# leonsick/s2d

Measured on AMD Instinct MI355X. Metric: clip-frames/sec fwd+loss, R50 M2F-Video T=8 720p Q=100, higher is better.
Workload: dtype f32 (f16x3 MFMA for dense contractions); 1 GPU; KDVideoMaskFormer fwd+loss (student+teacher fwd, GT+KD VideoSetCriterion), c4: 2 clips/GPU x T=8 x 720x1280, Q=100, P=160000, N=10 sparse GT instances/clip, encoder dropout 0.3; clips_per_gpu=2, frames_per_clip=8, parallelism=dp1 (clips sharded, no collective), streams=2

## Files before the change

s2d_amd/csrc/loss.hip:

```cpp
#include "common.h"
#include "class_select.h"

namespace {

__device__ __forceinline__ uint64_t mix64(uint64_t z)
{
    z += 0x9E3779B97F4A7C15ull;
    z = (z ^ (z >> 30)) * 0xBF58476D1CE4E5B9ull;
    z = (z ^ (z >> 27)) * 0x94D049BB133111EBull;
    return z ^ (z >> 31);
}
__device__ __forceinline__ uint32_t hash32(uint32_t x)
{
    x ^= x >> 16; x *= 0x7feb352du; x ^= x >> 15; x *= 0x846ca68bu; x ^= x >> 16;
    return x;
}
__device__ __forceinline__ uint32_t rand_key(uint64_t seed, uint64_t stream)
{
    return (uint32_t)mix64(seed ^ mix64(stream * 0xD1342543DE82EF95ull));
}
__device__ __forceinline__ uint32_t rand_u_bits(uint32_t key, uint32_t i) { return hash32(key + i); }
__device__ __forceinline__ uint32_t rand_v_bits(uint32_t a)
{
    uint32_t b = a * 0x9E3779B1u;
// ... 48 lines not shown
        int c = 0;
        for (int j = 0; j < Q; ++j)
            if (keep[j] && c < Nmax) kept[b * Nmax + c++] = j;
        count[b] = c;
    }
}

__global__ __launch_bounds__(256) void kd_upsample_kernel(const float *__restrict__ ml, int ldq, int T, int hm, int wm, int H,
                                                          int W, int Nmax, const int *__restrict__ count,
                                                          const int *__restrict__ kept, uint8_t *__restrict__ tgt,
                                                          int *__restrict__ nonempty)
{
    __shared__ int kq[128];
    __shared__ unsigned int anyset[128];
    const int bt = blockIdx.z, b = bt / T, t = bt % T;
    const int Y = blockIdx.y, X = blockIdx.x * 256 + threadIdx.x;
    const int cnt = count[b];
    if (threadIdx.x < 128) {
        kq[threadIdx.x] = threadIdx.x < cnt ? kept[b * Nmax + threadIdx.x] : 0;
        anyset[threadIdx.x] = 0u;
    }
    __syncthreads();
    if (X < W) {
        float sy = ((float)hm / H) * (Y + 0.5f) - 0.5f; if (sy < 0.f) sy = 0.f;
        float sx = ((float)wm / W) * (X + 0.5f) - 0.5f; if (sx < 0.f) sx = 0.f;
        const int y0 = (int)sy, x0 = (int)sx, y1 = y0 + (y0 < hm - 1 ? 1 : 0), x1 = x0 + (x0 < wm - 1 ? 1 : 0);
        const float ly = sy - y0, lx = sx - x0, hy = 1.f - ly, hx = 1.f - lx;
        const float *fr = ml + ((long)b * T + t) * hm * wm * ldq;
        const float *r00 = fr + ((long)y0 * wm + x0) * ldq, *r01 = fr + ((long)y0 * wm + x1) * ldq;
        const float *r10 = fr + ((long)y1 * wm + x0) * ldq, *r11 = fr + ((long)y1 * wm + x1) * ldq;
        for (int k = 0; k < cnt; ++k) {
            const int q = kq[k];
            const float val = hy * (hx * r00[q] + lx * r01[q]) + ly * (hx * r10[q] + lx * r11[q]);
            const uint8_t m = val > 0.f ? 1 : 0;
            tgt[((((long)b * Nmax + k) * T + t) * H + Y) * W + X] = m;
            if (m) anyset[k] = 1u;
        }
    }
    __syncthreads();
    if (threadIdx.x < cnt && anyset[threadIdx.x]) nonempty[((long)b * Nmax + threadIdx.x) * T + t] = 1;
}

constexpr int KDT_H = 16, KDT_W = 256, KDT_SH = 8, KDT_SW = 72, KDT_KC = 8;
__global__ __launch_bounds__(256) void kd_upsample_tile_kernel(const float *__restrict__ ml, int ldq, int T, int hm, int wm, int H,
                                                               int W, int Nmax, const int *__restrict__ count,
                                                               const int *__restrict__ kept, uint8_t *__restrict__ tgt,
                                                               int *__restrict__ nonempty)
{
    __shared__ int kq[128];
    __shared__ unsigned int anyset[128];
    __shared__ float src[KDT_KC][KDT_SH][KDT_SW];
    const int bt = blockIdx.z, b = bt / T, t = bt % T;
    const int Y0 = blockIdx.y * KDT_H, X0 = blockIdx.x * KDT_W;
    const int cnt = count[b];
    if (threadIdx.x < 128) {
        kq[threadIdx.x] = threadIdx.x < cnt ? kept[b * Nmax + threadIdx.x] : 0;
        anyset[threadIdx.x] = 0u;
    }
    auto srcpos = [](int o, int n_out, int n_in, int &i0, int &i1, float &l) {
        float s = ((float)n_in / n_out) * (o + 0.5f) - 0.5f; if (s < 0.f) s = 0.f;
        i0 = (int)s; i1 = i0 + (i0 < n_in - 1 ? 1 : 0); l = s - i0;
    };
    int ya, yb_, xa, xb_; float dummy;
    srcpos(Y0, H, hm, ya, yb_, dummy);
    srcpos(X0, W, wm, xa, xb_, dummy);
    const float *fr = ml + ((long)b * T + t) * hm * wm * ldq;
    const int xg = X0 + 4 * (threadIdx.x & 63);
    int x0[4], x1[4]; float lx[4];
#pragma unroll
    for (int e = 0; e < 4; ++e) srcpos(min(xg + e, W - 1), W, wm, x0[e], x1[e], lx[e]);
    __syncthreads();
    for (int k0 = 0; k0 < cnt; k0 += KDT_KC) {
        const int kc = min(KDT_KC, cnt - k0);
        for (int i = threadIdx.x; i < KDT_SH * KDT_SW * KDT_KC; i += 256) {
            const int kk = i % KDT_KC, pix = i / KDT_KC, sx = pix % KDT_SW, sy = pix / KDT_SW;
            const int gy = min(ya + sy, hm - 1), gx = min(xa + sx, wm - 1);
            if (kk < kc) src[kk][sy][sx] = fr[((long)gy * wm + gx) * ldq + kq[k0 + kk]];
        }
        __syncthreads();
#pragma unroll
        for (int pss = 0; pss < 4; ++pss) {
            const int Y = Y0 + (threadIdx.x >> 6) + 4 * pss;
            if (Y >= H || xg >= W) continue;
            int y0, y1; float ly;
            srcpos(Y, H, hm, y0, y1, ly);
            const float hy = 1.f - ly;
            for (int kk = 0; kk < kc; ++kk) {
                unsigned int word = 0u;
#pragma unroll
                for (int e = 0; e < 4; ++e) {
                    const float hx = 1.f - lx[e];
                    const float val = hy * (hx * src[kk][y0 - ya][x0[e] - xa] + lx[e] * src[kk][y0 - ya][x1[e] - xa]) +
                                      ly * (hx * src[kk][y1 - ya][x0[e] - xa] + lx[e] * src[kk][y1 - ya][x1[e] - xa]);
                    word |= (val > 0.f ? 1u : 0u) << (8 * e);
                }
                *reinterpret_cast<unsigned int *>(tgt + ((((long)b * Nmax + k0 + kk) * T + t) * H + Y) * W + xg) = word;
                if (word) anyset[k0 + kk] = 1u;
            }
        }
        __syncthreads();
    }
    if (threadIdx.x < cnt && anyset[threadIdx.x]) atomicOr(&nonempty[((long)b * Nmax + threadIdx.x) * T + t], 1);
}

constexpr int NE_CHUNKS = 8;
__global__ __launch_bounds__(256) void nonempty_kernel(const uint8_t *__restrict__ tgt, const int *__restrict__ count, int Nmax,
                                                       int T, long HW, int *__restrict__ nonempty)
{
    const int plane = blockIdx.x;
    const int n = (plane / T) % Nmax, b = plane / (T * Nmax);
    if (n >= count[b]) return;
    const uint8_t *p = tgt + (long)plane * HW;
    int any = 0;
    const long n16 = HW / 16, per = (n16 + NE_CHUNKS - 1) / NE_CHUNKS;
    const long lo = blockIdx.y * per, hi = min(lo + per, n16);
    const uint4 *p4 = reinterpret_cast<const uint4 *>(p);
    for (long i = lo + threadIdx.x; i < hi; i += 256) {
        const uint4 v = p4[i];
        any |= (v.x | v.y | v.z | v.w) != 0u;
    }
    if (blockIdx.y == 0)
        for (long i = n16 * 16 + threadIdx.x; i < HW; i += 256) any |= p[i] != 0;
    any = __syncthreads_or(any);
    if (threadIdx.x == 0 && any) atomicOr(&nonempty[plane], 1);
}

struct LossParams {
    const float *ml;
    const uint8_t *tgt;
    const int *tgt_count;
    const int *nonempty;
    const int *idx_q, *idx_t;
    const int *n_match;
    const float *coords_over;
    const float *coords_rand;
    uint64_t seed;
    int NL, B, Q, ldq, T, hm, wm, H, W, Nmax, maxm, n_over, n_unc, n_rand, drop;
    float world_size;
    int *active, *rank;
    int *list;
    int *lcount;
    float *mq;
    unsigned int *hist;
    unsigned int *prefix;
    int *krem;
    unsigned int *tie;
    float *part;
    int chunks;
    float *xbuf;
    unsigned int *tpack;
    int bits_global;
    int xcap;
    int *pbound;
};

__device__ __forceinline__ uint64_t key_row(const LossParams &p, long rowid)
{
    if (p.NL == 0) return (uint64_t)rowid;
    const long per = (long)p.maxm * p.T;
    const long lb = rowid / per;
    return (uint64_t)(lb * ((long)p.Q * p.T) + (rowid - lb * per));
}

constexpr int PB_STRIDE = 9;
struct VRange {
    float v0, dv;
};

__global__ void row_prep_kernel(LossParams p)
{
    const int layer = blockIdx.x;
    const int rows_l = p.B * p.maxm * p.T;
    __shared__ int base;
    if (threadIdx.x == 0) base = 0;
    __syncthreads();
    for (int r0 = 0; r0 < rows_l; r0 += blockDim.x) {
        const int r = r0 + threadIdx.x;
        int act = 0;
        if (r < rows_l) {
            const int t = r % p.T, s = (r / p.T) % p.maxm, b = r / (p.T * p.maxm);
            const int prob = layer * p.B + b;
            if (s < p.n_match[prob]) {
                const int n = p.idx_t[(long)prob * p.maxm + s];
                act = p.drop ? p.nonempty[((long)b * p.Nmax + n) * p.T + t] : 1;
            }
        }
        __shared__ int wsum[4];
        const unsigned long long m = __ballot(act);
        const int lane = threadIdx.x & 63, wv = threadIdx.x >> 6;
        const int inw = __popcll(m & ((1ull << lane) - 1ull));
        if (lane == 0) wsum[wv] = __popcll(m);
        __syncthreads();
        int off = base;
        for (int w = 0; w < wv; ++w) off += wsum[w];
        if (r < rows_l) {
            const long rowid = (long)layer * rows_l + r;
            p.active[rowid] = act;
            p.rank[rowid] = off + inw;
        }
        __syncthreads();
        if (threadIdx.x == 0) base += wsum[0] + wsum[1] + wsum[2] + wsum[3];
        __syncthreads();
    }
    if (threadIdx.x == 0) p.lcount[layer] = base;
}

__global__ void row_list_kernel(LossParams p)
{
    const int layer = blockIdx.x;
    const int rows_l = p.B * p.maxm * p.T;
    int base = 0;
    for (int l = 0; l < layer; ++l) base += p.lcount[l];
    for (int r = threadIdx.x; r < rows_l; r += blockDim.x) {
        const long rowid = (long)layer * rows_l + r;
        if (p.active[rowid]) p.list[base + p.rank[rowid]] = (int)rowid;
    }
    if (layer == p.NL - 1 && threadIdx.x == 0) p.lcount[p.NL] = base + p.lcount[layer];
}

__device__ int binomial_inv(int N, double p, double U);
__global__ __launch_bounds__(256) void row_strata_kernel(LossParams p, int nparts, int rpp)
{
    const int n = p.lcount[p.NL];
    const int wave = (blockIdx.x * 256 + threadIdx.x) >> 6, nwaves = gridDim.x * 4;
    for (int li = wave; li < n; li += nwaves) {
        const long rowid = p.list[li];
        int *pb = p.pbound + rowid * PB_STRIDE;
        int rem = p.n_over, at = 0;
        double mass = 1.0;
        for (int j = 0; j < nparts; ++j) {
            if ((threadIdx.x & 63) == 0) pb[j] = at;
            const double ya = j == 0 ? -0.5 : (double)(j * rpp), yb = j == nparts - 1 ? (double)p.hm - 0.5 : (double)((j + 1) * rpp);
            const double pj = (yb - ya) / (double)p.hm;
            int nj = rem;
            if (j < nparts - 1) {
                const uint64_t h = mix64(p.seed ^ mix64((key_row(p, rowid) * 16u + (uint64_t)j) * 0xD1342543DE82EF95ull + 0x5851F42D4C957F2Dull));
                const double U = (double)(h >> 11) * (1.0 / 9007199254740992.0);
                const double pc = pj / mass;
                nj = binomial_inv(rem, pc < 1.0 ? pc : 1.0, U);
            }
            at += nj; rem -= nj; mass -= pj;
        }
        if ((threadIdx.x & 63) == 0) pb[nparts] = at;
    }
}

__global__ void rng_points_prep_kernel(int *list, int nrows)
{
    const int i = blockIdx.x * 256 + threadIdx.x;
    if (i < nrows) list[i] = i;
    else if (i == nrows) list[i] = nrows;
}
__device__ __forceinline__ void over_point_rng(uint32_t key0, int i, const int *pb, const float *v0, const float *dv, int nparts, float &u, float &v);
__device__ __forceinline__ VRange part_vrange(int j, int nparts, int rpp, int hm);
__global__ void rng_points_kernel(LossParams p, int nparts, int rpp, float *__restrict__ uv)
{
    const int row = blockIdx.y, i = blockIdx.x * 256 + threadIdx.x;
    __shared__ float s_v0[PB_STRIDE], s_dv[PB_STRIDE];
    if ((int)threadIdx.x < nparts) { const VRange vr = part_vrange(threadIdx.x, nparts, rpp, p.hm); s_v0[threadIdx.x] = vr.v0; s_dv[threadIdx.x] = vr.dv; }
    __syncthreads();
    if (i >= p.n_over) return;
    float u, v;
    over_point_rng(rand_key(p.seed, (uint64_t)row * 2), i, p.pbound + (long)row * PB_STRIDE, s_v0, s_dv, nparts, u, v);
    uv[((long)row * p.n_over + i) * 2] = u;
    uv[((long)row * p.n_over + i) * 2 + 1] = v;
}

__global__ __launch_bounds__(256) void gather_rows_kernel(LossParams p)
{
    __shared__ float tile[64][129];
    const int prob = blockIdx.z, t = blockIdx.y, pix0 = blockIdx.x * 64;
    const int layer = prob / p.B, b = prob % p.B;
    const int hw = p.hm * p.wm;
    const int nm = p.n_match[prob];
    const long row_base = (((long)layer * p.B + b) * p.maxm) * p.T;
    bool any = false;
    for (int s = 0; s < nm; ++s) any = any || p.active[row_base + (long)s * p.T + t];
    if (!any) return;
    const float *src = p.ml + (((long)prob * p.T + t) * hw + pix0) * p.ldq;
    const int npix = min(64, hw - pix0);
    const int l4 = p.ldq >> 2;
    f32x4 v[8];
    const int tot = npix * l4;
#pragma unroll
    for (int k = 0; k < 8; ++k) {
        const int e = threadIdx.x + 256 * k;
        if (e < tot) v[k] = *reinterpret_cast<const f32x4 *>(src + (long)e * 4);
    }
#pragma unroll
    for (int k = 0; k < 8; ++k) {
        const int e = threadIdx.x + 256 * k;
        if (e < tot) {
            const int px = e / l4, q = (e - px * l4) * 4;
            if (q < 128) { tile[px][q] = v[k][0]; tile[px][q + 1] = v[k][1]; tile[px][q + 2] = v[k][2]; tile[px][q + 3] = v[k][3]; }
        }
    }
    __syncthreads();
    const int lane = threadIdx.x & 63, wv = threadIdx.x >> 6;
    for (int s = wv; s < nm; s += 4) {
        const long rowid = row_base + (long)s * p.T + t;
        if (!p.active[rowid]) continue;
        const int q = p.idx_q[(long)prob * p.maxm + s];
        if (lane < npix) p.mq[rowid * hw + pix0 + lane] = tile[lane][q];
    }
}

// ... 118 lines not shown
        reinterpret_cast<f32x4 *>(sm + (long)(nr + 1) * wp)[i] = z;
    }
    for (int i = threadIdx.x; i < nr; i += LTHREADS) {
        *reinterpret_cast<f32x4 *>(sm + (long)(i + 1) * wp) = z;
        *reinterpret_cast<f32x4 *>(sm + (long)(i + 1) * wp + PADC + wm) = z;
    }
    const f32x4 *src = reinterpret_cast<const f32x4 *>(map + (long)r0 * wm);
    for (int e = threadIdx.x; e < nr * w4; e += LTHREADS) {
        const int row = e / w4, c4 = e - row * w4;
        *reinterpret_cast<f32x4 *>(sm + (long)(row + 1) * wp + PADC + 4 * c4) = src[e];
    }
}

__device__ __forceinline__ float sample_part_padded(const float *__restrict__ sm, int wp, int r0, float x, float y, int x0, int y0)
{
    const float fx = x - x0, fy = y - y0;
    const float *b = sm + (y0 - r0 + 1) * wp + x0 + PADC;
    float acc = b[0] * ((1.f - fx) * (1.f - fy));
    acc += b[1] * (fx * (1.f - fy));
    acc += b[wp] * ((1.f - fx) * fy);
    acc += b[wp + 1] * (fx * fy);
    return acc;
}

__device__ __forceinline__ float sample_part(const float *__restrict__ sm, int hm, int wm, int r0, int nr, float x, float y, int x0, int y0)
{
    const int x1 = x0 + 1, y1 = y0 + 1;
    const float fx = x - x0, fy = y - y0;
    const float wxa = (x0 >= 0) ? 1.f - fx : 0.f, wxb = (x1 < wm) ? fx : 0.f;
    const float wya = (y0 >= 0) ? 1.f - fy : 0.f, wyb = (y1 < hm) ? fy : 0.f;
    const int xa = max(x0, 0), xb = min(x1, wm - 1);
    const int ya = min(max(y0 - r0, 0), nr - 1) * wm, yb = min(max(min(y1, hm - 1) - r0, 0), nr - 1) * wm;
    float acc = sm[ya + xa] * (wxa * wya);
    acc += sm[ya + xb] * (wxb * wya);
    acc += sm[yb + xa] * (wxa * wyb);
    acc += sm[yb + xb] * (wxb * wyb);
    return acc;
}

#ifndef S2D_LOSS_DBG
#define S2D_LOSS_DBG 0
#endif
template <int LEVEL>
__global__ __launch_bounds__(LTHREADS) void hist_kernel(LossParams p)
{
    extern __shared__ __attribute__((aligned(16))) float smem[];
    __shared__ int hq_idx[LTHREADS / 64][128];
    __shared__ float hq_y[LTHREADS / 64][128];
    constexpr int nb = LEVEL == 0 ? 2048 : 1024;
    const PartGeom g = part_geom(p.hm, p.wm);
    unsigned int *h = reinterpret_cast<unsigned int *>(smem);
    float *sm = smem + 2048;
    PartIter it(p, g.nparts, LEVEL == 0 ? 0 : p.xcap);
    long rowid; int part, li;
    while (it.next(p, rowid, part, li)) {
        __syncthreads();
        for (int i = threadIdx.x; i < nb; i += LTHREADS) h[i] = 0u;
        const int r0 = part * g.rows_per_part;
        const int nr = min(g.rows_per_part + 1, p.hm - r0);
        const float *cr = coord_rows(p, rowid, true);
        const bool padded = cr == nullptr;
        const int wp = p.wm + 2 * PADC;
        if (padded) stage_part_padded(p.mq + rowid * p.hm * p.wm, p.wm, r0, nr, sm);
        else stage_part(p.mq + rowid * p.hm * p.wm, p.wm, r0, nr, sm);
        __syncthreads();
        const unsigned int pre = LEVEL > 0 ? p.prefix[rowid] : 0u;
        const uint32_t key0 = rand_key(p.seed, key_row(p, rowid) * 2);
        const int ylo = part == 0 ? -1 : r0, yhi = r0 + g.rows_per_part;
        auto tally = [&](int i, float xv) {
            const unsigned int key = __float_as_uint(fabsf(xv));
            if (LEVEL == 0 && li < p.xcap && !(S2D_LOSS_DBG & 4)) p.xbuf[(long)li * (p.n_over + p.n_rand) + i] = xv;
            if ((S2D_LOSS_DBG & 1) && LEVEL == 0) { if (key == 0x12345u) h[0] = 1u; return; }
            if (LEVEL == 0) atomicAdd(&h[key >> 20], 1u);
            else if (LEVEL == 1) { if ((key >> 20) == (pre >> 20)) atomicAdd(&h[(key >> 10) & 1023u], 1u); }
            else { if ((key >> 10) == (pre >> 10)) atomicAdd(&h[key & 1023u], 1u); }
        };
        if (!cr) {
            const int *pb = p.pbound + rowid * PB_STRIDE;
            const int lo = pb[part], hi = pb[part + 1];
            const VRange vr = part_vrange(part, g.nparts, g.rows_per_part, p.hm);
            const int y0max = min(yhi, p.hm) - 1;
#pragma unroll 2
            for (int i = lo + (int)threadIdx.x; i < hi; i += LTHREADS) {
                const uint32_t ra_ = rand_u_bits(key0, (uint32_t)i);
                const float u = (float)(ra_ >> 8) * (1.0f / 16777216.0f);
                const float v = fmaf((float)(rand_v_bits(ra_) >> 8) * (1.0f / 16777216.0f), vr.dv, vr.v0);
                const float y = ((2.f * v - 1.f + 1.f) * p.hm - 1.f) * 0.5f;
                const float x = ((2.f * u - 1.f + 1.f) * p.wm - 1.f) * 0.5f;
                const int y0 = min(max((int)floorf(y), ylo), y0max);
                if (S2D_LOSS_DBG & 2) tally(i, x * y + (float)y0); else
                tally(i, sample_part_padded(sm, wp, r0, x, y, (int)floorf(x), y0));
            }
        } else {
            const int lane = threadIdx.x & 63, wv = threadIdx.x >> 6;
            int *qi = hq_idx[wv];
            float *qy = hq_y[wv];
            int qn = 0;
            auto heavy = [&](int i, float y) {
                const float u = cr[2 * i];
                const float x = ((2.f * u - 1.f + 1.f) * p.wm - 1.f) * 0.5f;
                tally(i, sample_part(sm, p.hm, p.wm, r0, nr, x, y, (int)floorf(x), (int)floorf(y)));
            };
            const int iters = (p.n_over + LTHREADS - 1) / LTHREADS;
            for (int k = 0; k < iters; ++k) {
                const int i = k * LTHREADS + threadIdx.x;
                const bool live = i < p.n_over;
                const int ic = live ? i : p.n_over - 1;
                const float v = cr[2 * ic + 1];
                const float y = ((2.f * v - 1.f + 1.f) * p.hm - 1.f) * 0.5f;
                const int y0 = (int)floorf(y);
                const bool own = live && y0 >= ylo && y0 < yhi;
                const unsigned long long m = __ballot(own);
                if (own) {
                    const int pos = qn + (int)__popcll(m & ((1ull << lane) - 1ull));
                    qi[pos] = i; qy[pos] = y;
                }
                qn += (int)__popcll(m);
                if (qn >= 64) {
                    heavy(qi[lane], qy[lane]);
                    const int rest = qn - 64;
                    int ti = 0; float ty = 0.f;
                    if (lane < rest) { ti = qi[64 + lane]; ty = qy[64 + lane]; }
                    if (lane < rest) { qi[lane] = ti; qy[lane] = ty; }
                    qn = rest;
                }
            }
            if (lane < qn) heavy(qi[lane], qy[lane]);
        }
        if (LEVEL == 0 && li < p.xcap) {
            const float *cr2 = coord_rows(p, rowid, false);
            const uint32_t key1 = rand_key(p.seed, key_row(p, rowid) * 2 + 1);
            for (int i = threadIdx.x; i < p.n_rand; i += LTHREADS) {
                float u, v;
                if (cr2) { u = cr2[2 * i]; v = cr2[2 * i + 1]; }
                else {
                    const uint32_t ra_ = rand_u_bits(key1, (uint32_t)i);
                    u = (float)(ra_ >> 8) * (1.0f / 16777216.0f);
                    v = (float)(rand_v_bits(ra_) >> 8) * (1.0f / 16777216.0f);
                }
                const float y = ((2.f * v - 1.f + 1.f) * p.hm - 1.f) * 0.5f;
                const float x = ((2.f * u - 1.f + 1.f) * p.wm - 1.f) * 0.5f;
                const int y0 = (int)floorf(y);
                if (y0 >= ylo && y0 < yhi)
                    p.xbuf[(long)li * (p.n_over + p.n_rand) + p.n_over + i] =
                        padded ? sample_part_padded(sm, wp, r0, x, y, (int)floorf(x), y0) : sample_part(sm, p.hm, p.wm, r0, nr, x, y, (int)floorf(x), y0);
            }
        }
        __syncthreads();
        for (int i = threadIdx.x; i < nb; i += LTHREADS)
            if (h[i]) atomicAdd(&p.hist[rowid * 2048 + i], h[i]);
    }
}

template <int LEVEL>
__global__ __launch_bounds__(256) void hist_stream_kernel(LossParams p)
{
    __shared__ unsigned int h[1024];
    constexpr int SCH = 8;
    const int nrows = min(p.lcount[p.NL], p.xcap);
    for (int w = blockIdx.x; w < nrows * SCH; w += gridDim.x) {
        const int li = w / SCH, chunk = w % SCH;
        const long rowid = p.list[li];
        __syncthreads();
        for (int i = threadIdx.x; i < 1024; i += 256) h[i] = 0u;
        __syncthreads();
        const unsigned int pre = p.prefix[rowid];
        const float *xb = p.xbuf + (long)li * (p.n_over + p.n_rand);
        const int per = ((p.n_over + SCH - 1) / SCH + 3) & ~3;
        const int i0 = chunk * per, i1 = min(p.n_over, i0 + per);
        for (int i = i0 + threadIdx.x * 4; i < i1; i += 256 * 4) {
            const f32x4 v = *reinterpret_cast<const f32x4 *>(xb + i);
#pragma unroll
            for (int j = 0; j < 4; ++j) {
                if (i + j >= i1) break;
                const unsigned int key = __float_as_uint(fabsf(v[j]));
                if (LEVEL == 1) { if ((key >> 20) == (pre >> 20)) atomicAdd(&h[(key >> 10) & 1023u], 1u); }
                else { if ((key >> 10) == (pre >> 10)) atomicAdd(&h[key & 1023u], 1u); }
            }
        }
        __syncthreads();
        for (int i = threadIdx.x; i < 1024; i += 256)
            if (h[i]) atomicAdd(&p.hist[rowid * 2048 + i], h[i]);
    }
}

template <bool COH = false>
__device__ __forceinline__ float sample_bits(const unsigned int *bits, int H, int W, float u, float v)
{
    const float gx = 2.f * u - 1.f, gy = 2.f * v - 1.f;
    const float x = ((gx + 1.f) * W - 1.f) * 0.5f, y = ((gy + 1.f) * H - 1.f) * 0.5f;
    const int x0 = (int)floorf(x), y0 = (int)floorf(y), x1 = x0 + 1, y1 = y0 + 1;
    const float fx = x - x0, fy = y - y0;
    const float wxa = (x0 >= 0 && x0 < W) ? 1.f - fx : 0.f, wxb = (x1 >= 0 && x1 < W) ? fx : 0.f;
    const float wya = (y0 >= 0 && y0 < H) ? 1.f - fy : 0.f, wyb = (y1 >= 0 && y1 < H) ? fy : 0.f;
    const int xa = min(max(x0, 0), W - 1), xb = min(max(x1, 0), W - 1);
    const int ya = min(max(y0, 0), H - 1) * W, yb = min(max(y1, 0), H - 1) * W;
    auto bit = [&](int idx) {
        const unsigned int w = COH ? __hip_atomic_load(bits + (idx >> 5), __ATOMIC_RELAXED, __HIP_MEMORY_SCOPE_AGENT) : bits[idx >> 5];
        return (float)((w >> (idx & 31)) & 1u);
    };
    float acc = bit(ya + xa) * (wxa * wya);
    acc += bit(ya + xb) * (wxb * wya);
    acc += bit(yb + xa) * (wxa * wyb);
    acc += bit(yb + xb) * (wxb * wyb);
    return acc;
}

template <int LEVEL>
__global__ __launch_bounds__(256) void select_kernel(LossParams p)
{
    __shared__ unsigned int csum[256];
    if ((int)blockIdx.x >= p.lcount[p.NL]) return;
    const long rowid = p.list[blockIdx.x];
    const int nb = LEVEL == 0 ? 2048 : 1024, per = nb / 256;
    const int k = LEVEL == 0 ? p.n_unc : p.krem[rowid];
    unsigned int *h = p.hist + rowid * 2048;
    unsigned int loc[8], s = 0;
    for (int j = 0; j < per; ++j) { loc[j] = h[threadIdx.x * per + j]; s += loc[j]; }
    csum[threadIdx.x] = s;
    __syncthreads();
    if (threadIdx.x == 0) {
        unsigned int run = 0;
        for (int i = 0; i < 256; ++i) { const unsigned int c = csum[i]; csum[i] = run; run += c; }
    }
    __syncthreads();
    unsigned int before = csum[threadIdx.x];
    if (k == 0 && LEVEL == 0 && threadIdx.x == 0) { p.prefix[rowid] = 0u; p.krem[rowid] = 0; }
    for (int j = 0; j < per; ++j) {
        if (before < (unsigned)k && before + loc[j] >= (unsigned)k) {
            const unsigned int bin = threadIdx.x * per + j;
            const unsigned int pre = LEVEL == 0 ? 0u : p.prefix[rowid];
            p.prefix[rowid] = LEVEL == 0 ? (bin << 20) : LEVEL == 1 ? (pre | (bin << 10)) : (pre | bin);
            p.krem[rowid] = k - (int)before;
        }
        before += loc[j];
    }
    __syncthreads();
    for (int j = 0; j < per; ++j) h[threadIdx.x * per + j] = 0u;
}

__device__ __forceinline__ void acc_point(float x, float t, float &bce, float &sgt, float &sg, float &ts)
{
    const float e = __expf(-fabsf(x));
    const float inv = __builtin_amdgcn_rcpf(1.f + e);
    const float s = x >= 0.f ? inv : e * inv;
    bce += fmaxf(x, 0.f) - x * t + __logf(1.f + e);
    sgt += s * t; sg += s; ts += t;
}

__global__ __launch_bounds__(LTHREADS) void accumulate_kernel(LossParams p)
{
    extern __shared__ __attribute__((aligned(16))) float smem[];
    __shared__ float red[LTHREADS / 64][4];
    const PartGeom g = part_geom(p.hm, p.wm);
    float *sm = smem;
    const int rows_l = p.B * p.maxm * p.T;
    PartIter it(p, g.nparts, p.xcap);
    long rowid; int part, li;
    while (it.next(p, rowid, part, li)) {
        __syncthreads();
        const int r0 = part * g.rows_per_part;
        const int nr = min(g.rows_per_part + 1, p.hm - r0);
        stage_part(p.mq + rowid * p.hm * p.wm, p.wm, r0, nr, sm);
        __syncthreads();
        const int layer = (int)(rowid / rows_l);
        const int r = (int)(rowid % rows_l);
        const int t = r % p.T, s = (r / p.T) % p.maxm, b = r / (p.T * p.maxm);
        const int prob = layer * p.B + b;
        const int n = p.idx_t[(long)prob * p.maxm + s];
        const uint8_t *pl = p.tgt + (((long)b * p.Nmax + n) * p.T + t) * p.H * p.W;
        const unsigned int thr = p.prefix[rowid];
        const unsigned int take = (unsigned int)p.krem[rowid];
        const int ylo = part == 0 ? -1 : r0, yhi = r0 + g.rows_per_part;
        float bce = 0.f, sgt = 0.f, sg = 0.f, ts = 0.f;
#pragma unroll 1
        for (int pass = 0; pass < 2; ++pass) {
            const bool over = pass == 0;
            const float *cr = coord_rows(p, rowid, over);
            const uint32_t key0 = rand_key(p.seed, key_row(p, rowid) * 2 + (over ? 0 : 1));
            const bool strat = over && !cr;
            const int *pb = p.pbound + rowid * PB_STRIDE;
            const int ibeg = strat ? pb[part] : 0, cnt = strat ? pb[part + 1] : (over ? p.n_over : p.n_rand);
            const VRange vr = part_vrange(part, g.nparts, g.rows_per_part, p.hm);
            const int y0max = min(yhi, p.hm) - 1;
            for (int i0 = ibeg + (int)threadIdx.x; i0 < cnt; i0 += 4 * LTHREADS) {
                float xv[4], uu[4], vv[4];
                bool own[4];
#pragma unroll
                for (int j = 0; j < 4; ++j) {
                    const int i = i0 + j * LTHREADS;
                    const int ic = min(i, cnt - 1);
                    float u, v;
                    if (cr) { u = cr[2 * ic]; v = cr[2 * ic + 1]; }
                    else {
                        const uint32_t ra_ = rand_u_bits(key0, (uint32_t)ic);
                        u = (float)(ra_ >> 8) * (1.0f / 16777216.0f);
                        v = (float)(rand_v_bits(ra_) >> 8) * (1.0f / 16777216.0f);
                        if (strat) v = fmaf(v, vr.dv, vr.v0);
                    }
                    const float y = ((2.f * v - 1.f + 1.f) * p.hm - 1.f) * 0.5f;
                    const float x = ((2.f * u - 1.f + 1.f) * p.wm - 1.f) * 0.5f;
                    int y0 = (int)floorf(y);
                    if (strat) y0 = min(max(y0, ylo), y0max);
                    own[j] = i < cnt && y0 >= ylo && y0 < yhi;
                    xv[j] = sample_part(sm, p.hm, p.wm, r0, nr, x, y, (int)floorf(x), y0);
                    uu[j] = u; vv[j] = v;
                }
#pragma unroll
                for (int j = 0; j < 4; ++j) {
                    bool sel = own[j];
                    if (over && sel) {
                        const unsigned int key = __float_as_uint(fabsf(xv[j]));
                        sel = key < thr;
                        if (key == thr) sel = atomicAdd(&p.tie[rowid], 1u) < take;
                    }
                    if (sel) acc_point(xv[j], sample_plane(pl, p.H, p.W, uu[j], vv[j]), bce, sgt, sg, ts);
                }
            }
        }
        bce = wave_sum(bce); sgt = wave_sum(sgt); sg = wave_sum(sg); ts = wave_sum(ts);
        const int lane = threadIdx.x & 63, wv = threadIdx.x >> 6;
        if (lane == 0) { red[wv][0] = bce; red[wv][1] = sgt; red[wv][2] = sg; red[wv][3] = ts; }
        __syncthreads();
        if (threadIdx.x < 4) {
            const int j = threadIdx.x;
            float tot = 0.f;
#pragma unroll
            for (int w = 0; w < LTHREADS / 64; ++w) tot += red[w][j];
            p.part[(rowid * p.chunks + part) * 4 + j] = tot;
        }
    }
}

__global__ __launch_bounds__(256) void pack_planes_kernel(LossParams p)
{
    const long HW = (long)p.H * p.W, wpp = HW / 32;
    const int plane = blockIdx.y;
    const int n = (plane / p.T) % p.Nmax, b = plane / (p.T * p.Nmax);
    if (n >= min(p.tgt_count[b], p.Nmax)) return;
    const long wd = (long)blockIdx.x * 256 + threadIdx.x;
    if (wd >= wpp) return;
    const uint8_t *pl = p.tgt + (long)plane * HW;
    const uint4 a = reinterpret_cast<const uint4 *>(pl)[wd * 2], c = reinterpret_cast<const uint4 *>(pl)[wd * 2 + 1];
    const unsigned int ws[8] = {a.x, a.y, a.z, a.w, c.x, c.y, c.z, c.w};
    unsigned int out = 0u;
#pragma unroll
    for (int k = 0; k < 8; ++k) {
        const unsigned int w4 = ws[k];
        out |= ((w4 & 0xFFu) ? 1u : 0u) << (4 * k);
        out |= ((w4 & 0xFF00u) ? 1u : 0u) << (4 * k + 1);
        out |= ((w4 & 0xFF0000u) ? 1u : 0u) << (4 * k + 2);
        out |= ((w4 & 0xFF000000u) ? 1u : 0u) << (4 * k + 3);
    }
    p.tpack[(long)plane * wpp + wd] = out;
}

struct LossBwdArgs {
    float *gplane;
    float w_mask, w_dice;
    unsigned int *bit_scratch;
};
template <bool BWD, bool GBITS = BWD>
__global__ __launch_bounds__(LTHREADS) void accumulate_stream_kernel(LossParams p, LossBwdArgs ba)
{
    extern __shared__ __attribute__((aligned(16))) unsigned int tbits[];
    __shared__ float red[LTHREADS / 64][4];
    constexpr int TIECAP = 512;
    __shared__ unsigned int tie_n, tie_base, wtie[LTHREADS / 64];
    __shared__ int tie_idx[TIECAP], tie_sorted[TIECAP];
    __shared__ int cq_idx[LTHREADS / 64][128];
    __shared__ float cq_val[LTHREADS / 64][128];
    const int rows_l = p.B * p.maxm * p.T;
    const int nrows = min(p.lcount[p.NL], p.xcap);
    const long HW = (long)p.H * p.W;
    __shared__ float s_v0[PB_STRIDE], s_dv[PB_STRIDE];
    __shared__ int s_pb[PB_STRIDE];
    const PartGeom sg_ = part_geom(p.hm, p.wm);
    if ((int)threadIdx.x < sg_.nparts) { const VRange vr = part_vrange(threadIdx.x, sg_.nparts, sg_.rows_per_part, p.hm); s_v0[threadIdx.x] = vr.v0; s_dv[threadIdx.x] = vr.dv; }
    static_assert(GBITS || !BWD, "the backward keeps its gradient tile in the dynamic LDS");
    const unsigned int *tb = tbits;
    int *gh = reinterpret_cast<int *>(tbits);
    const float n_pts = (float)(p.n_unc + p.n_rand);
    const bool injected = p.coords_over != nullptr || p.coords_rand != nullptr;
    const float FX_CAP = injected ? fmaxf(n_pts, 1.f) : fminf(fmaxf(n_pts, 1.f), fmaxf(1024.f, 256.f * n_pts / (float)(p.hm * p.wm)));
    __shared__ unsigned int tie_before;
    for (int li = blockIdx.x; li < nrows; li += gridDim.x) {
        const long rowid = p.list[li];
        const int layer = (int)(rowid / rows_l);
        const int r = (int)(rowid % rows_l);
        const int t = r % p.T, s = (r / p.T) % p.maxm, b = r / (p.T * p.maxm);
// ... 360 lines not shown
        if (threadIdx.x < n_match[b]) matched[idx_q[(long)b * maxm + threadIdx.x]] = 1;
        __syncthreads();
        const int q = threadIdx.x;
        if (q < Q) {
            const float *l = cls + ((long)b * Q + q) * C1;
            float mx, sum;
            softmax_row_stats(l, C1, mx, sum);
            const float lse = mx + logf(sum);
            const bool m = matched[q];
            const float w = m ? 1.f : eos;
            num += (double)(w * (lse - (m ? l[0] : l[C1 - 1])));
            den += (double)w;
        }
    }
    num = wave_sum_d(num); den = wave_sum_d(den);
    if ((threadIdx.x & 63) == 0) { wnum[threadIdx.x >> 6] = num; wden[threadIdx.x >> 6] = den; }
    __syncthreads();
    if (threadIdx.x == 0) {
        double sn = 0., sd = 0.;
        for (unsigned int w = 0; w < (blockDim.x + 63) / 64; ++w) { sn += wnum[w]; sd += wden[w]; }
        out[0] = (float)(sn / sd);
    }
}

__global__ __launch_bounds__(256) void class_loss_backward_c_kernel(const float *__restrict__ cls, int C1, const int *__restrict__ idx_q,
                                                                    const int *__restrict__ n_match, int B, int Q, int maxm, float eos,
                                                                    float w_ce, float *__restrict__ dcls)
{
    __shared__ unsigned char matched[128];
    __shared__ float mxs[128], sums[128];
    const int b = blockIdx.x;
    double den = 0.;
    for (int bb = 0; bb < B; ++bb) den += (double)n_match[bb] + (double)eos * (Q - n_match[bb]);
    const float wsum = (float)den;
    if (threadIdx.x < 128) matched[threadIdx.x] = 0;
    __syncthreads();
    if ((int)threadIdx.x < n_match[b]) matched[idx_q[(long)b * maxm + threadIdx.x]] = 1;
    if ((int)threadIdx.x < Q) {
        float mx, sum;
        softmax_row_stats(cls + ((long)b * Q + threadIdx.x) * C1, C1, mx, sum);
        mxs[threadIdx.x] = mx; sums[threadIdx.x] = sum;
    }
    __syncthreads();
    const long n = (long)Q * C1;
    for (long i = threadIdx.x; i < n; i += 256) {
        const int q = (int)(i / C1), c = (int)(i - (long)q * C1);
        const float e = expf(cls[(long)b * n + i] - mxs[q]);
        const float pc = e / sums[q];
        const bool m = matched[q];
        const float w = (m ? 1.f : eos) * w_ce / wsum;
        const float onehot = (c == (m ? 0 : C1 - 1)) ? 1.f : 0.f;
        dcls[(long)b * n + i] = w * (pc - onehot);
    }
}

__global__ __launch_bounds__(256) void kd_compact_kernel(const int *__restrict__ rank, int n, int C, int K, int Nmax, int *__restrict__ count,
                                                         int *__restrict__ kept, int *__restrict__ label)
{
    __shared__ int wcnt[4];
    const int b = blockIdx.x, lane = threadIdx.x & 63, w = threadIdx.x >> 6;
    int base = 0;
    for (int j0 = 0; j0 < n; j0 += 256) {
        const int i = j0 + threadIdx.x;
        const bool keep = i < n && rank[(long)b * n + i] < K;
        const unsigned long long bal = __ballot(keep);
        const int before = __popcll(bal & ((1ull << lane) - 1ull));
        __syncthreads();
        if (lane == 0) wcnt[w] = __popcll(bal);
        __syncthreads();
        int off = base + before;
        for (int v = 0; v < w; ++v) off += wcnt[v];
        if (keep && off < Nmax) {
            kept[(long)b * Nmax + off] = i / C;
            label[(long)b * Nmax + off] = i % C;
        }
        base += wcnt[0] + wcnt[1] + wcnt[2] + wcnt[3];
    }
    if (threadIdx.x == 0) count[b] = base < Nmax ? base : Nmax;
}

}

static int kd_upsample_launch(const float *t_mask_logits, int B, int ldq, int T, int hm, int wm, int H, int W, int Nmax, uint8_t *tgt,
                              const int *count, const int *kept_q, int *nonempty, hipStream_t stream)
{
    if (W % 4 == 0 && (reinterpret_cast<uintptr_t>(tgt) & 3) == 0 && 16L * hm + 2L * H <= (long)KDT_SH * H && 256L * wm + 2L * W <= (long)KDT_SW * W)
        hipLaunchKernelGGL(kd_upsample_tile_kernel, dim3(cdiv(W, KDT_W), cdiv(H, KDT_H), B * T), dim3(256), 0, stream, t_mask_logits, ldq, T, hm, wm,
                           H, W, Nmax, count, kept_q, tgt, nonempty);
    else
        hipLaunchKernelGGL(kd_upsample_kernel, dim3(cdiv(W, 256), H, B * T), dim3(256), 0, stream, t_mask_logits, ldq, T, hm, wm,
                           H, W, Nmax, count, kept_q, tgt, nonempty);
    S2D_CHECK_LAUNCH();
    return S2D_OK;
}

extern "C" {

int s2d_kd_targets_u8(const float *t_class_logits, const float *t_mask_logits, float score_thr, int topk, int B, int Q,
                      int ldq, int T, int hm, int wm, int H, int W, int Nmax, uint8_t *tgt, int *count, int *kept_q,
                      int *nonempty, hipStream_t stream)
{
    if (Q > 128 || Nmax > 128) return S2D_ERR_ARG;
    if (B == 0) return S2D_OK;
    if (s2d_zero_async(nonempty, sizeof(int) * (size_t)B * Nmax * T, stream) != S2D_OK) return S2D_ERR_LAUNCH;
    hipLaunchKernelGGL(kd_select_kernel, dim3(B), dim3(128), 0, stream, t_class_logits, Q, topk < Q ? topk : Q, score_thr,
                       Nmax, count, kept_q);
    return kd_upsample_launch(t_mask_logits, B, ldq, T, hm, wm, H, W, Nmax, tgt, count, kept_q, nonempty, stream);
}

long s2d_kd_targets_c_workspace_bytes(int B, int Q, int C1)
{
    return C1 < 2 ? 0 : cls_select_workspace_bytes(B, Q, C1);
}

int s2d_kd_targets_c_u8(const float *t_class_logits, int C1, const float *t_mask_logits, float score_thr, int topk, int B, int Q,
                        int ldq, int T, int hm, int wm, int H, int W, int Nmax, void *workspace, uint8_t *tgt, int *count, int *kept_q,
                        int *label, int *nonempty, hipStream_t stream)
{
    if (Q > 128 || Nmax > 128 || C1 < 2 || topk < 0 || (long)Q * (C1 - 1) > 0x7FFFFFFFL / 2) return S2D_ERR_ARG;
    if (B == 0) return S2D_OK;
    const int n = Q * (C1 - 1);
    if (s2d_zero_async(nonempty, sizeof(int) * (size_t)B * Nmax * T, stream) != S2D_OK) return S2D_ERR_LAUNCH;
    int *rank = nullptr;
    cls_select_launch(t_class_logits, B, Q, C1, topk < n ? topk : n, score_thr, workspace, &rank, nullptr, nullptr, nullptr, stream);
    hipLaunchKernelGGL(kd_compact_kernel, dim3(B), dim3(256), 0, stream, rank, n, C1 - 1, topk < n ? topk : n, Nmax, count, kept_q, label);
    return kd_upsample_launch(t_mask_logits, B, ldq, T, hm, wm, H, W, Nmax, tgt, count, kept_q, nonempty, stream);
}


int s2d_target_nonempty(const uint8_t *tgt, const int *count, int B, int Nmax, int T, int H, int W, int *nonempty,
                        hipStream_t stream)
{
    if (B * Nmax * T == 0) return S2D_OK;
    if (((long)H * W) % 16) return S2D_ERR_ARG;
    if (s2d_zero_async(nonempty, sizeof(int) * (size_t)B * Nmax * T, stream) != S2D_OK) return S2D_ERR_LAUNCH;
    hipLaunchKernelGGL(nonempty_kernel, dim3(B * Nmax * T, NE_CHUNKS), dim3(256), 0, stream, tgt, count, Nmax, T, (long)H * W, nonempty);
    S2D_CHECK_LAUNCH();
    return S2D_OK;
}

static const int LOSS_CHUNKS = 8;

static const long XBUF_MAX_ROWS = 4096;

static void point_counts(int num_points, float oversample_ratio, float importance_ratio, int &n_over, int &n_unc, int &n_rand)
{
    n_over = (int)(num_points * oversample_ratio);
    n_unc = (int)(importance_ratio * num_points);
    n_rand = num_points - n_unc;
}

static inline bool plane_in_lds(long HW) { return HW / 8 <= 140 * 1024; }
constexpr int ACC_BLOCKS = 512;

long s2d_point_loss_workspace_bytes(int NL, int B, int Q, int Nmax, int T, int hm, int wm, int num_points,
                                    float oversample_ratio, float importance_ratio, int H, int W)
{
    const long maxm = Q < Nmax ? Q : Nmax;
    const long rows = (long)NL * B * maxm * T;
    int n_over, n_unc, n_rand;
    point_counts(num_points, oversample_ratio, importance_ratio, n_over, n_unc, n_rand);
    const long xrows = rows < XBUF_MAX_ROWS ? rows : XBUF_MAX_ROWS;
    const long HW = (long)H * W;
    return rows * (3 * 4 + (long)hm * wm * 4 + 2048 * 4 + 4 + 4 + 4 + LOSS_CHUNKS * 16 + PB_STRIDE * 4) + 4L * (NL + 1) + 1024 +
           xrows * (long)(n_over + n_rand + 8) * 4 + 256 + (long)B * Nmax * T * (HW / 32 + 1) * 4;
}

static int loss_setup(LossParams &p, long &rows, const float *mask_logits, const uint8_t *tgt, const int *tgt_count, const int *nonempty,
                      const int *idx_q, const int *idx_t, const int *n_match, const float *coords_over, const float *coords_rand,
                      uint64_t seed, int NL, int B, int Q, int ldq, int T, int hm, int wm, int H, int W, int Nmax, int num_points,
                      float oversample_ratio, float importance_ratio, int drop_empty, float world_size, void *workspace)
{
    if (Q > 128 || Nmax > 128 || ldq > 128 || ldq < Q || (ldq & 3)) return S2D_ERR_ARG;
    p.ml = mask_logits; p.tgt = tgt; p.tgt_count = tgt_count; p.nonempty = nonempty;
    p.idx_q = idx_q; p.idx_t = idx_t; p.n_match = n_match; p.coords_over = coords_over; p.coords_rand = coords_rand;
    p.seed = seed; p.NL = NL; p.B = B; p.Q = Q; p.ldq = ldq; p.T = T; p.hm = hm; p.wm = wm; p.H = H; p.W = W; p.Nmax = Nmax;
    p.maxm = Q < Nmax ? Q : Nmax;
    point_counts(num_points, oversample_ratio, importance_ratio, p.n_over, p.n_unc, p.n_rand);
    p.drop = drop_empty; p.world_size = world_size; p.chunks = LOSS_CHUNKS;
    rows = (long)NL * B * p.maxm * T;
    if (rows == 0) return S2D_OK;
    char *w = (char *)workspace;
    p.active = (int *)w; w += rows * 4;
    p.rank = (int *)w; w += rows * 4;
    p.prefix = (unsigned int *)w; w += rows * 4;
    p.krem = (int *)w; w += rows * 4;
    p.tie = (unsigned int *)w; w += rows * 4;
    p.list = (int *)w; w += rows * 4;
    p.lcount = (int *)w; w += 4L * (NL + 1);
    w = (char *)(((uintptr_t)w + 255) & ~(uintptr_t)255);
    p.hist = (unsigned int *)w; w += rows * 2048 * 4;
    p.part = (float *)w; w += rows * LOSS_CHUNKS * 16;
    p.pbound = (int *)w; w += rows * PB_STRIDE * 4;
    p.mq = (float *)w; w += rows * (long)hm * wm * 4;
    w = (char *)(((uintptr_t)w + 255) & ~(uintptr_t)255);
    p.xbuf = (float *)w;
    const bool can_stream = (p.n_over % 4 == 0) && (p.n_rand % 4 == 0) && ((long)H * W % 32 == 0);
    p.xcap = can_stream ? (int)(rows < XBUF_MAX_ROWS ? rows : XBUF_MAX_ROWS) : 0;
    {
        char *e = (char *)p.xbuf + (long)(rows < XBUF_MAX_ROWS ? rows : XBUF_MAX_ROWS) * (p.n_over + p.n_rand + 8) * 4;
        p.tpack = (unsigned int *)(((uintptr_t)e + 255) & ~(uintptr_t)255);
    }
    p.bits_global = can_stream && !plane_in_lds((long)H * W);
    const PartGeom pg = part_geom(hm, wm);
    if ((wm & 3) || pg.rows_per_part < 1 || pg.nparts > LOSS_CHUNKS) return S2D_ERR_ARG;
    p.chunks = pg.nparts;
    return S2D_OK;
}

static int loss_attrs()
{
    static S2dDevOnce attr_set;
    if (!attr_set.done()) {
        const int cap = PART_BYTES + 8192 + 4096;
        if (hipFuncSetAttribute(reinterpret_cast<const void *>(hist_kernel<0>), hipFuncAttributeMaxDynamicSharedMemorySize, cap) != hipSuccess ||
            hipFuncSetAttribute(reinterpret_cast<const void *>(hist_kernel<1>), hipFuncAttributeMaxDynamicSharedMemorySize, cap) != hipSuccess ||
            hipFuncSetAttribute(reinterpret_cast<const void *>(hist_kernel<2>), hipFuncAttributeMaxDynamicSharedMemorySize, cap) != hipSuccess ||
            hipFuncSetAttribute(reinterpret_cast<const void *>(accumulate_kernel), hipFuncAttributeMaxDynamicSharedMemorySize, cap) != hipSuccess ||
            hipFuncSetAttribute(reinterpret_cast<const void *>(accumulate_stream_kernel<false>), hipFuncAttributeMaxDynamicSharedMemorySize, 140 * 1024) != hipSuccess ||
            hipFuncSetAttribute(reinterpret_cast<const void *>(accumulate_stream_kernel<false, true>), hipFuncAttributeMaxDynamicSharedMemorySize, 140 * 1024) != hipSuccess ||
            hipFuncSetAttribute(reinterpret_cast<const void *>(accumulate_stream_kernel<true>), hipFuncAttributeMaxDynamicSharedMemorySize, 140 * 1024) != hipSuccess)
            return S2D_ERR_LAUNCH;
        attr_set.mark();
    }
    return S2D_OK;
}

int s2d_point_loss_f32(const float *mask_logits, const uint8_t *tgt, const int *tgt_count, const int *nonempty,
                       const int *idx_q, const int *idx_t, const int *n_match, const float *coords_over,
                       const float *coords_rand, uint64_t seed, int NL, int B, int Q, int ldq, int T, int hm, int wm, int H,
                       int W, int Nmax, int num_points, float oversample_ratio, float importance_ratio, int drop_empty,
                       float world_size, void *workspace, float *losses, hipStream_t stream)
{
    LossParams p;
    long rows = 0;
    if (int e = loss_setup(p, rows, mask_logits, tgt, tgt_count, nonempty, idx_q, idx_t, n_match, coords_over, coords_rand, seed, NL, B, Q, ldq,
                           T, hm, wm, H, W, Nmax, num_points, oversample_ratio, importance_ratio, drop_empty, world_size, workspace))
        return e;
    if (rows == 0) return S2D_OK;
    if (s2d_zero_async(p.hist, (size_t)rows * 2048 * 4, stream) != S2D_OK) return S2D_ERR_LAUNCH;
    if (s2d_zero_async(p.tie, (size_t)rows * 4, stream) != S2D_OK) return S2D_ERR_LAUNCH;
    hipLaunchKernelGGL(row_prep_kernel, dim3(NL), dim3(256), 0, stream, p);
    hipLaunchKernelGGL(row_list_kernel, dim3(NL), dim3(256), 0, stream, p);
    hipLaunchKernelGGL(gather_rows_kernel, dim3(cdiv((long)hm * wm, 64), T, NL * B), dim3(256), 0, stream, p);
    const PartGeom pg = part_geom(hm, wm);
    static_assert(PB_STRIDE == LOSS_CHUNKS + 1, "one bound per part + the end");
    if (!coords_over) hipLaunchKernelGGL(row_strata_kernel, dim3(cdiv(rows, 4)), dim3(256), 0, stream, p, pg.nparts, pg.rows_per_part);
    const size_t lds_map = sizeof(float) * (size_t)(pg.rows_per_part + 3) * (wm + 2 * PADC);
    const size_t lds_hist = lds_map + sizeof(float) * 2048;
    if (int e = loss_attrs()) return e;
    const dim3 g(512);
    hipLaunchKernelGGL(hist_kernel<0>, g, dim3(LTHREADS), lds_hist, stream, p);
    hipLaunchKernelGGL(select_kernel<0>, dim3((unsigned)rows), dim3(256), 0, stream, p);
    if (p.xcap > 0) hipLaunchKernelGGL(hist_stream_kernel<1>, dim3(2048), dim3(256), 0, stream, p);
    if (rows > p.xcap) hipLaunchKernelGGL(hist_kernel<1>, g, dim3(LTHREADS), lds_hist, stream, p);
    hipLaunchKernelGGL(select_kernel<1>, dim3((unsigned)rows), dim3(256), 0, stream, p);
    if (p.xcap > 0) hipLaunchKernelGGL(hist_stream_kernel<2>, dim3(2048), dim3(256), 0, stream, p);
    if (rows > p.xcap) hipLaunchKernelGGL(hist_kernel<2>, g, dim3(LTHREADS), lds_hist, stream, p);
    hipLaunchKernelGGL(select_kernel<2>, dim3((unsigned)rows), dim3(256), 0, stream, p);
    if (p.xcap > 0)
        hipLaunchKernelGGL(pack_planes_kernel, dim3(cdiv((long)H * W / 32, 256), B * Nmax * T), dim3(256), 0, stream, p);
    if (p.xcap > 0 && !p.bits_global)
        hipLaunchKernelGGL(accumulate_stream_kernel<false>, dim3(ACC_BLOCKS), dim3(LTHREADS), (size_t)((long)H * W / 8), stream, p, LossBwdArgs{nullptr, 0.f, 0.f, nullptr});
    else if (p.xcap > 0)
        hipLaunchKernelGGL((accumulate_stream_kernel<false, true>), dim3(ACC_BLOCKS), dim3(LTHREADS), 16, stream, p, LossBwdArgs{nullptr, 0.f, 0.f, nullptr});
    if (rows > p.xcap) hipLaunchKernelGGL(accumulate_kernel, g, dim3(LTHREADS), lds_map, stream, p);
    hipLaunchKernelGGL(loss_finalize_kernel, dim3(NL), dim3(64), 0, stream, p, losses);
    S2D_CHECK_LAUNCH();
    return S2D_OK;
}

int s2d_point_loss_backward_f32(const float *mask_logits, const uint8_t *tgt, const int *tgt_count, const int *nonempty,
                                const int *idx_q, const int *idx_t, const int *n_match, const float *coords_over,
                                const float *coords_rand, uint64_t seed, int NL, int B, int Q, int ldq, int T, int hm, int wm, int H,
                                int W, int Nmax, int num_points, float oversample_ratio, float importance_ratio, int drop_empty,
                                float world_size, void *workspace, float w_mask, float w_dice, float *grad_rows,
                                unsigned int *bit_scratch, hipStream_t stream)
{
    LossParams p;
    long rows = 0;
    if (int e = loss_setup(p, rows, mask_logits, tgt, tgt_count, nonempty, idx_q, idx_t, n_match, coords_over, coords_rand, seed, NL, B, Q, ldq,
                           T, hm, wm, H, W, Nmax, num_points, oversample_ratio, importance_ratio, drop_empty, world_size, workspace))
        return e;
    if (rows == 0) return S2D_OK;
    if (p.xcap <= 0) return S2D_ERR_ARG;
    if (int e = loss_attrs()) return e;
    if (s2d_zero_async(grad_rows, sizeof(float) * (size_t)rows * hm * wm, stream) != S2D_OK) return S2D_ERR_LAUNCH;
    const PartGeom pg = part_geom(hm, wm);
    const size_t lds = sizeof(int) * (size_t)(pg.rows_per_part + 3 < hm ? pg.rows_per_part + 3 : hm) * wm;
    if (lds > 140 * 1024 || 3L * wm > 4L * LTHREADS || pg.nparts + 1 > PB_STRIDE) return S2D_ERR_ARG;
    hipLaunchKernelGGL(accumulate_stream_kernel<true>, dim3(ACC_BLOCKS), dim3(LTHREADS), lds, stream, p,
                       LossBwdArgs{grad_rows, w_mask, w_dice, bit_scratch});
    S2D_CHECK_LAUNCH();
    return S2D_OK;
}

int s2d_point_loss_rng_points(uint64_t seed, int hm, int wm, int row0, int nrows, int n_over, float *uv, int *bounds, int *scratch_list,
                              hipStream_t stream)
{
    const PartGeom pg = part_geom(hm, wm);
    if ((wm & 3) || pg.rows_per_part < 1 || pg.nparts > LOSS_CHUNKS || nrows <= 0 || row0 != 0) return S2D_ERR_ARG;
    LossParams p = {};
    p.seed = seed; p.hm = hm; p.wm = wm; p.n_over = n_over; p.NL = 0;
    p.list = scratch_list;
    p.lcount = scratch_list + nrows;
    p.pbound = bounds;
    hipLaunchKernelGGL(rng_points_prep_kernel, dim3(cdiv(nrows + 1, 256)), dim3(256), 0, stream, scratch_list, nrows);
    hipLaunchKernelGGL(row_strata_kernel, dim3(cdiv(nrows, 4)), dim3(256), 0, stream, p, pg.nparts, pg.rows_per_part);
    hipLaunchKernelGGL(rng_points_kernel, dim3(cdiv(n_over, 256), nrows), dim3(256), 0, stream, p, pg.nparts, pg.rows_per_part, uv);
    S2D_CHECK_LAUNCH();
    return S2D_OK;
}

int s2d_class_loss_backward_f32(const float *class_logits, const int *idx_q, const int *n_match, int B, int Q, int maxm, float eos_coef,
                                float w_ce, float *d_class_logits, hipStream_t stream)
{
    if (Q > 128) return S2D_ERR_ARG;
    hipLaunchKernelGGL(class_loss_backward_kernel, dim3(1), dim3(128), 0, stream, class_logits, idx_q, n_match, B, Q, maxm, eos_coef, w_ce,
                       d_class_logits);
    S2D_CHECK_LAUNCH();
    return S2D_OK;
}

int s2d_class_loss_f32(const float *class_logits, const int *idx_q, const int *n_match, int B, int Q, int maxm,
                       float eos_coef, float *loss_ce, hipStream_t stream)
{
    if (Q > 128) return S2D_ERR_ARG;
    hipLaunchKernelGGL(class_loss_kernel, dim3(1), dim3(128), 0, stream, class_logits, idx_q, n_match, B, Q, maxm, eos_coef,
                       loss_ce);
    S2D_CHECK_LAUNCH();
    return S2D_OK;
}

int s2d_class_loss_c_f32(const float *class_logits, int C1, const int *idx_q, const int *n_match, int B, int Q, int maxm,
                         float eos_coef, float *loss_ce, hipStream_t stream)
{
    if (Q > 128 || C1 < 2) return S2D_ERR_ARG;
    hipLaunchKernelGGL(class_loss_c_kernel, dim3(1), dim3(128), 0, stream, class_logits, C1, idx_q, n_match, B, Q, maxm, eos_coef,
                       loss_ce);
    S2D_CHECK_LAUNCH();
    return S2D_OK;
}

int s2d_class_loss_backward_c_f32(const float *class_logits, int C1, const int *idx_q, const int *n_match, int B, int Q, int maxm,
                                  float eos_coef, float w_ce, float *d_class_logits, hipStream_t stream)
{
    if (Q > 128 || C1 < 2) return S2D_ERR_ARG;
    if (B == 0) return S2D_OK;
    hipLaunchKernelGGL(class_loss_backward_c_kernel, dim3(B), dim3(256), 0, stream, class_logits, C1, idx_q, n_match, B, Q, maxm,
                       eos_coef, w_ce, d_class_logits);
    S2D_CHECK_LAUNCH();
    return S2D_OK;
}

// ... 2 lines not shown
```

Before: 176.0 clip-frames/s.

## Compact level-1 radix candidates to skip level-2 streaming histogram pass

During the second radix-select histogram pass over the oversampled point logits, keys that match the level-0 prefix are compacted per wavefront into a global candidate buffer when the selected bucket count fits a capacity of n_over/8. The level-2 select kernel then builds its histogram from this small candidate list in LDS, and the level-2 streaming pass skips those rows entirely. This removes a full re-read of xbuf for most rows, at the cost of extra ballot/LDS queue work, atomics on a fill counter, and additional workspace.

```diff
diff --git a/s2d_amd/csrc/loss.hip b/s2d_amd/csrc/loss.hip
--- a/s2d_amd/csrc/loss.hip
+++ b/s2d_amd/csrc/loss.hip
@@ -224,6 +224,10 @@
     int bits_global;
     int xcap;
     int *pbound;
+    unsigned int *bcount;
+    unsigned int *cfill;
+    unsigned int *cand;
+    int ccap;
 };
 
 __device__ __forceinline__ uint64_t key_row(const LossParams &p, long rowid)
@@ -648,15 +652,21 @@
     }
 }
 
+constexpr int CQ_CAP = 512;
 template <int LEVEL>
 __global__ __launch_bounds__(256) void hist_stream_kernel(LossParams p)
 {
     __shared__ unsigned int h[1024];
+    __shared__ unsigned int cq[LEVEL == 1 ? 4 : 1][LEVEL == 1 ? CQ_CAP : 1];
     constexpr int SCH = 8;
     const int nrows = min(p.lcount[p.NL], p.xcap);
+    const int lane = threadIdx.x & 63, wv = threadIdx.x >> 6;
     for (int w = blockIdx.x; w < nrows * SCH; w += gridDim.x) {
         const int li = w / SCH, chunk = w % SCH;
         const long rowid = p.list[li];
+        const unsigned int bc = p.bcount[rowid];
+        if (LEVEL == 2 && bc <= (unsigned int)p.ccap) continue;
+        const bool compact = LEVEL == 1 && bc > 0u && bc <= (unsigned int)p.ccap;
         __syncthreads();
         for (int i = threadIdx.x; i < 1024; i += 256) h[i] = 0u;
         __syncthreads();
@@ -664,14 +674,50 @@
         const float *xb = p.xbuf + (long)li * (p.n_over + p.n_rand);
         const int per = ((p.n_over + SCH - 1) / SCH + 3) & ~3;
         const int i0 = chunk * per, i1 = min(p.n_over, i0 + per);
-        for (int i = i0 + threadIdx.x * 4; i < i1; i += 256 * 4) {
-            const f32x4 v = *reinterpret_cast<const f32x4 *>(xb + i);
-#pragma unroll
-            for (int j = 0; j < 4; ++j) {
-                if (i + j >= i1) break;
-                const unsigned int key = __float_as_uint(fabsf(v[j]));
-                if (LEVEL == 1) { if ((key >> 20) == (pre >> 20)) atomicAdd(&h[(key >> 10) & 1023u], 1u); }
-                else { if ((key >> 10) == (pre >> 10)) atomicAdd(&h[key & 1023u], 1u); }
+        if (LEVEL == 1) {
+            unsigned int *q = cq[wv];
+            unsigned int *cd = p.cand + (long)li * p.ccap;
+            int qn = 0;
+            auto flush = [&]() {
+                unsigned int base = 0u;
+                if (lane == 0) base = atomicAdd(&p.cfill[rowid], (unsigned int)qn);
+                base = __shfl(base, 0);
+                for (int k = lane; k < qn; k += 64)
+                    if (base + k < (unsigned int)p.ccap) cd[base + k] = q[k];
+                qn = 0;
+            };
+            for (int ib = i0; ib < i1; ib += 256 * 4) {
+                const int i = ib + threadIdx.x * 4;
+                f32x4 v = {0.f, 0.f, 0.f, 0.f};
+                if (i < i1) v = *reinterpret_cast<const f32x4 *>(xb + i);
+                unsigned int key[4];
+                bool in[4];
+#pragma unroll
+                for (int j = 0; j < 4; ++j) {
+                    key[j] = __float_as_uint(fabsf(v[j]));
+                    in[j] = i + j < i1 && (key[j] >> 20) == (pre >> 20);
+                    if (in[j]) atomicAdd(&h[(key[j] >> 10) & 1023u], 1u);
+                }
+                if (compact) {
+#pragma unroll
+                    for (int j = 0; j < 4; ++j) {
+                        const unsigned long long m = __ballot(in[j]);
+                        if (in[j]) q[qn + (int)__popcll(m & ((1ull << lane) - 1ull))] = key[j];
+                        qn += (int)__popcll(m);
+                    }
+                    if (qn >= CQ_CAP - 256) flush();
+                }
+            }
+            if (compact && qn > 0) flush();
+        } else {
+            for (int i = i0 + threadIdx.x * 4; i < i1; i += 256 * 4) {
+                const f32x4 v = *reinterpret_cast<const f32x4 *>(xb + i);
+#pragma unroll
+                for (int j = 0; j < 4; ++j) {
+                    if (i + j >= i1) break;
+                    const unsigned int key = __float_as_uint(fabsf(v[j]));
+                    if ((key >> 10) == (pre >> 10)) atomicAdd(&h[key & 1023u], 1u);
+                }
             }
         }
         __syncthreads();
@@ -706,13 +752,32 @@
 __global__ __launch_bounds__(256) void select_kernel(LossParams p)
 {
     __shared__ unsigned int csum[256];
+    __shared__ unsigned int hc[LEVEL == 2 ? 1024 : 1];
+    __shared__ unsigned int s_bc;
     if ((int)blockIdx.x >= p.lcount[p.NL]) return;
     const long rowid = p.list[blockIdx.x];
     const int nb = LEVEL == 0 ? 2048 : 1024, per = nb / 256;
     const int k = LEVEL == 0 ? p.n_unc : p.krem[rowid];
     unsigned int *h = p.hist + rowid * 2048;
+    if (LEVEL == 0 && threadIdx.x == 0) s_bc = 0u;
+    bool fromc = false;
+    if (LEVEL == 2 && (int)blockIdx.x < p.xcap) {
+        const unsigned int n = p.bcount[rowid];
+        fromc = n <= (unsigned int)p.ccap;
+        if (fromc) {
+            for (int i = threadIdx.x; i < 1024; i += 256) hc[i] = 0u;
+            __syncthreads();
+            const unsigned int pre = p.prefix[rowid];
+            const unsigned int *cd = p.cand + (long)blockIdx.x * p.ccap;
+            for (unsigned int i = threadIdx.x; i < n; i += 256) {
+                const unsigned int key = cd[i];
+                if ((key >> 10) == (pre >> 10)) atomicAdd(&hc[key & 1023u], 1u);
+            }
+            __syncthreads();
+        }
+    }
     unsigned int loc[8], s = 0;
-    for (int j = 0; j < per; ++j) { loc[j] = h[threadIdx.x * per + j]; s += loc[j]; }
+    for (int j = 0; j < per; ++j) { loc[j] = (LEVEL == 2 && fromc) ? hc[threadIdx.x * per + j] : h[threadIdx.x * per + j]; s += loc[j]; }
     csum[threadIdx.x] = s;
     __syncthreads();
     if (threadIdx.x == 0) {
@@ -728,10 +793,13 @@
             const unsigned int pre = LEVEL == 0 ? 0u : p.prefix[rowid];
             p.prefix[rowid] = LEVEL == 0 ? (bin << 20) : LEVEL == 1 ? (pre | (bin << 10)) : (pre | bin);
             p.krem[rowid] = k - (int)before;
+            if (LEVEL == 0) s_bc = loc[j];
         }
         before += loc[j];
     }
     __syncthreads();
+    if (LEVEL == 0 && threadIdx.x == 0) { p.bcount[rowid] = s_bc; p.cfill[rowid] = 0u; }
+    if (fromc) return;
     for (int j = 0; j < per; ++j) h[threadIdx.x * per + j] = 0u;
 }
 
@@ -1398,6 +1466,7 @@
 
 static inline bool plane_in_lds(long HW) { return HW / 8 <= 140 * 1024; }
 constexpr int ACC_BLOCKS = 512;
+static inline int cand_cap(int n_over) { return n_over / 8; }
 
 long s2d_point_loss_workspace_bytes(int NL, int B, int Q, int Nmax, int T, int hm, int wm, int num_points,
                                     float oversample_ratio, float importance_ratio, int H, int W)
@@ -1409,7 +1478,8 @@
     const long xrows = rows < XBUF_MAX_ROWS ? rows : XBUF_MAX_ROWS;
     const long HW = (long)H * W;
     return rows * (3 * 4 + (long)hm * wm * 4 + 2048 * 4 + 4 + 4 + 4 + LOSS_CHUNKS * 16 + PB_STRIDE * 4) + 4L * (NL + 1) + 1024 +
-           xrows * (long)(n_over + n_rand + 8) * 4 + 256 + (long)B * Nmax * T * (HW / 32 + 1) * 4;
+           xrows * (long)(n_over + n_rand + 8) * 4 + 256 + (long)B * Nmax * T * (HW / 32 + 1) * 4 +
+           512 + rows * 8 + xrows * (long)cand_cap(n_over) * 4;
 }
 
 static int loss_setup(LossParams &p, long &rows, const float *mask_logits, const uint8_t *tgt, const int *tgt_count, const int *nonempty,
@@ -1446,6 +1516,12 @@
     {
         char *e = (char *)p.xbuf + (long)(rows < XBUF_MAX_ROWS ? rows : XBUF_MAX_ROWS) * (p.n_over + p.n_rand + 8) * 4;
         p.tpack = (unsigned int *)(((uintptr_t)e + 255) & ~(uintptr_t)255);
+        e = (char *)p.tpack + (long)B * Nmax * T * ((long)H * W / 32 + 1) * 4;
+        e = (char *)(((uintptr_t)e + 255) & ~(uintptr_t)255);
+        p.bcount = (unsigned int *)e; e += rows * 4;
+        p.cfill = (unsigned int *)e; e += rows * 4;
+        p.cand = (unsigned int *)(((uintptr_t)e + 255) & ~(uintptr_t)255);
+        p.ccap = cand_cap(p.n_over);
     }
     p.bits_global = can_stream && !plane_in_lds((long)H * W);
     const PartGeom pg = part_geom(hm, wm);
```

New measurement: 176.0 clip-frames/s (median of 3 runs). About the same (-0.0%).
